# cafferychen777/flashdeconv

Measured on AMD Instinct MI355X. Metric: spots/sec to convergence (1M x 2000 x 30), higher is better.
Workload: dtype f64

## Files before the change

### flashdeconv_amd/csrc/bcd_sweep_inst.cpp

```cpp
#include <algorithm>
#include <cstdlib>
#include "bcd_device.h"
#include "fdx_graph.h"

#ifndef FDX_PART
#error "compile with -DFDX_PART=<n> -DFDX_K_LO=<lo> -DFDX_K_HI=<hi>"
#endif

namespace fdx {

constexpr int sweep_chunk(int K) {
#ifdef FDX_KC_OVERRIDE
    return K < FDX_KC_OVERRIDE ? K : FDX_KC_OVERRIDE;
#endif
    return K < 8 ? K : K <= 29 ? 8 : K <= 33 ? 7 : K <= 37 ? 6 : K <= 41 ? 5 : K <= 45 ? 4 : K <= 49 ? 3 : K <= 51 ? 2 : K <= 64 ? 8 : K <= 72 ? 6 : K <= 88 ? 4 : K <= 96 ? 2 : 8;
}

template <int K, int KC>
__global__ __launch_bounds__(256) void bcd_sweep_kernel(
    const double* __restrict__ H, const double* __restrict__ XtX, const double* __restrict__ beta_in,
    double* __restrict__ beta_out, const int* __restrict__ ell_base, const int* __restrict__ slice_off,
    const int* __restrict__ deg, unsigned long long* __restrict__ stats, double* __restrict__ rel_change,
    const double lambda, const double rho, const double tol, const int ldh, const int ld_, const int n,
    const int n_slices, const int it) {
    const int lane = threadIdx.x & 63;
    const int wib = __builtin_amdgcn_readfirstlane(threadIdx.x >> 6);

    if (it > 0) {
        const double rc = fold_rel_change(stats + (size_t)(it - 1) * 128, lane);
        if (blockIdx.x == 0 && threadIdx.x == 0) rel_change[it - 1] = rc;
        if (rc < tol) return;
    }

    const int slice = xcd_remap(blockIdx.x, gridDim.x) * 4 + wib;
    if (slice >= n_slices) return;
    const int i = min(slice * 64 + lane, n - 1);
    const size_t ld = (size_t)ld_;

    const int w0 = slice_off[slice];
    const int w = slice_off[slice + 1] - w0;

    double b[K];
#pragma unroll
    for (int k = 0; k < K; ++k) b[k] = beta_in[k * ld + i];
    const int* ell = ell_base + (size_t)w0 * 64 + (i & 63);
    const int dg = deg[i];
    const double lam_deg = lambda * (double)dg;
    const double lam_eff = (dg > 0) ? lambda : 0.0;

    double dmax = 0.0, amax = 0.0;
#pragma unroll
    for (int kc = 0; kc < K; kc += KC) {
        double c[KC];
#pragma unroll
        for (int q = 0; q < KC; ++q) c[q] = 0.0;
#pragma unroll 2
        for (int m = 0; m < w; ++m) {
            const int j = ell[(size_t)m * 64];
#pragma unroll
            for (int q = 0; q < KC; ++q)
                if (kc + q < K) c[q] += beta_in[(kc + q) * ld + j];
        }
#pragma unroll
        for (int q = 0; q < KC; ++q) {
            const int k = kc + q;
            if (k < K) {
                const double h = H[k * (size_t)ldh + i];
                const double* g = XtX + k * K;
                double r0 = 0.0, r1 = 0.0;
#pragma unroll
                for (int j = 0; j + 1 < K; j += 2) {
                    r0 = fma(g[j], b[j], r0);
                    r1 = fma(g[j + 1], b[j + 1], r1);
                }
                if (K & 1) r0 = fma(g[K - 1], b[K - 1], r0);
                const double gkk = g[k];
                const double old = b[k];
                const double res = (h - (r0 + r1) + gkk * old) + lam_eff * c[q];
                const double den = gkk + lam_deg;
                const double st = res > rho ? res - rho : (res < -rho ? res + rho : 0.0);
                const double qv = fmax(0.0, st / den);
                const double nw = (den > 1e-10) ? qv : 0.0;
                dmax = fmax(dmax, fabs(nw - old));
                amax = fmax(amax, fabs(old));
                b[k] = nw;
                beta_out[k * ld + i] = nw;
            }
        }
    }
    dmax = wave_max(dmax);
    amax = wave_max(amax);
    if (lane == 0) {
        unsigned long long* s = stats + (size_t)it * 128;
        const int slot = slice & 63;
        atomicMax(s + slot, (unsigned long long)__double_as_longlong(dmax));
        atomicMax(s + 64 + slot, (unsigned long long)__double_as_longlong(amax));
    }
}

__device__ __forceinline__ const char __attribute__((address_space(1)))* plane_base(const double* p) {
    unsigned long long v = (unsigned long long)p;
    asm("" : "+s"(v));
    return (const char __attribute__((address_space(1)))*)v;
}

__device__ __forceinline__ unsigned lane_off(unsigned off) {
    asm("" : "+v"(off));
    return off;
}

#ifndef FDX_SWEEP_WPE
#define FDX_SWEEP_WPE 1
#endif
template <int K, int KC, bool OBJ, bool QUAD = true, bool INIT = false>
__global__ __launch_bounds__(256, ((OBJ && K > 40 && K <= 64) || (K > 64 && K <= 96)) ? 2 : (OBJ ? 1 : FDX_SWEEP_WPE)) void bcd_sweep_tiled_kernel(
    const double* __restrict__ H, const double* __restrict__ XtX, const double* __restrict__ beta_in,
    double* __restrict__ beta_out, const unsigned short* __restrict__ ell_local, const int* __restrict__ slice_off,
    const int* __restrict__ deg, const int* __restrict__ tile_halo, const int* __restrict__ tile_hcnt,
    unsigned long long* __restrict__ stats, double* __restrict__ rel_change, const double lambda, const double rho,
    const double tol, const int ldh, const int ld_, const int n, const int S, const int it,
    const int* __restrict__ tile_list, const double init_v, const int* __restrict__ send_head, const int4* __restrict__ send_ent,
    double* __restrict__ send_buf) {
    extern __shared__ __attribute__((aligned(16))) double lds[];
    const int tid = threadIdx.x;
    const int lane = tid & 63;
    const int tile = tile_list ? tile_list[xcd_remap(blockIdx.x, gridDim.x)] : xcd_remap(blockIdx.x, gridDim.x);
    const bool real = (tile * 256 + tid) < n;
    const int i = min(tile * 256 + tid, n - 1);
    const size_t ld = (size_t)ld_;
    const int slice = __builtin_amdgcn_readfirstlane(i >> 6);
    const int w0 = slice_off[slice];
    const int w = slice_off[slice + 1] - w0;
    const int Ht = tile_hcnt[tile];
    const int* halo = tile_halo + (size_t)tile * FDX_TILE_HALO_CAP;
    const int dg = deg[i];
    int hidx0 = halo[tid];
    if (!OBJ && it > 0) {
        const double rc = fold_rel_change(stats + (size_t)(it - 1) * 128, lane);
        if (blockIdx.x == 0 && tid == 0) rel_change[it - 1] = rc;
        asm volatile("" :: "v"(dg), "v"(hidx0), "s"(w0), "s"(w), "s"(Ht));
        if (rc < tol) return;
    }
    hidx0 = (tid < Ht) ? hidx0 : 0;

    const unsigned ioff = (unsigned)i * 8u, hoff = (unsigned)hidx0 * 8u;
#define PLANE_AT(base, off) (*(const double __attribute__((address_space(1)))*)(plane_base(base) + lane_off(off)))
    double b[K];
#pragma unroll
    for (int k = 0; k < K; ++k) b[k] = INIT ? init_v : PLANE_AT(beta_in + k * ld, ioff);
    const unsigned short* ell = ell_local + (size_t)w0 * 64 + (i & 63);
    const double lam_deg = lambda * (double)dg;
    const double lam_eff = (dg > 0) ? lambda : 0.0;
    unsigned slots[8];
    const unsigned zslot = (unsigned)(256 + Ht);
#pragma unroll
    for (int m2 = 0; m2 < 8; ++m2) {
        unsigned lo = (unsigned)__builtin_nontemporal_load(&ell[(size_t)(2 * m2) * 64]);
        unsigned hi = (unsigned)__builtin_nontemporal_load(&ell[(size_t)(2 * m2 + 1) * 64]);
        lo = (2 * m2 < w) ? lo : zslot;
        hi = (2 * m2 + 1 < w) ? hi : zslot;
        slots[m2] = lo | (hi << 16);
    }
    double hv[KC], hreg[KC];
#pragma unroll
    for (int q = 0; q < KC; ++q) {
        hv[q] = INIT ? init_v : PLANE_AT(beta_in + q * ld, hoff);
        hreg[q] = __builtin_nontemporal_load(&PLANE_AT(H + q * (size_t)ldh, ioff));
    }

    double dmax = 0.0, amax = 0.0;
    double o_cross = 0.0, o_quad = 0.0, o_spat = 0.0, o_l1 = 0.0;
#pragma unroll
    for (int kc = 0; kc < K; kc += KC) {
#pragma unroll
        for (int q = 0; q < KC; ++q)
            if (kc + q < K) lds[q * S + tid] = b[kc + q];
        if (tid < Ht) {
#pragma unroll
            for (int q = 0; q < KC; ++q)
                if (kc + q < K) lds[q * S + 256 + tid] = hv[q];
        }
        for (int h = tid + 256; h < Ht; h += 256) {
            const int j = halo[h];
#pragma unroll
            for (int q = 0; q < KC; ++q)
                if (kc + q < K) lds[q * S + 256 + h] = INIT ? init_v : beta_in[(kc + q) * ld + j];
        }
        if (tid < KC) lds[tid * S + 256 + Ht] = 0.0;
        __syncthreads();
        double c[KC];
#pragma unroll
        for (int q = 0; q < KC; ++q) c[q] = 0.0;
#pragma unroll
        for (int m4 = 0; m4 < 16; m4 += 4) {
            if (m4 < w) {
#pragma unroll
                for (int m = m4; m < m4 + 4; ++m) {
                    const int slot = (int)((slots[m >> 1] >> (16 * (m & 1))) & 0xffffu);
#pragma unroll
                    for (int q = 0; q < KC; ++q)
                        if (kc + q < K) c[q] += lds[q * S + slot];
                }
            }
        }
        for (int m = 16; m < w; ++m) {
            const int slot = ell[(size_t)m * 64];
#pragma unroll
            for (int q = 0; q < KC; ++q)
                if (kc + q < K) c[q] += lds[q * S + slot];
        }
        __syncthreads();
#pragma unroll
        for (int q = 0; q < KC; ++q) {
            const int k = kc + q;
            if (k < K) {
                const double h = hreg[q];
                const double* g = XtX + k * K;
                double r0 = 0.0, r1 = 0.0;
                if (!OBJ || QUAD) {
#pragma unroll
                    for (int j = 0; j + 1 < K; j += 2) {
                        r0 = fma(g[j], b[j], r0);
                        r1 = fma(g[j + 1], b[j + 1], r1);
                    }
                    if (K & 1) r0 = fma(g[K - 1], b[K - 1], r0);
                }
                const double gkk = (!OBJ || QUAD) ? g[k] : 0.0;
                const double old = b[k];
                if (OBJ) {
                    o_cross = fma(old, h, o_cross);
                    if (QUAD) o_quad = fma(old, r0 + r1, o_quad);
                    o_spat = fma(old, (double)dg * old - c[q], o_spat);
                    o_l1 += fabs(old);
                    asm volatile("" : "+v"(o_quad));
                } else {
                    const double res = (h - (r0 + r1) + gkk * old) + lam_eff * c[q];
                    const double den = gkk + lam_deg;
                    const double st = res > rho ? res - rho : (res < -rho ? res + rho : 0.0);
                    const double qv = fmax(0.0, st / den);
                    const double nw = (den > 1e-10) ? qv : 0.0;
                    dmax = fmax(dmax, fabs(nw - old));
                    amax = fmax(amax, fabs(old));
                    b[k] = nw;
                    __builtin_nontemporal_store(nw, (double __attribute__((address_space(1)))*)(plane_base(beta_out + k * ld) + lane_off(ioff)));
                }
            }
            if (kc + KC < K) {
#pragma unroll
                for (int t = 2 * q; t < 2 * q + 2; ++t) {
                    const int j = t < KC ? t : t - KC;
                    if (kc + KC + j < K) {
                        if (t < KC) { if (!INIT) hv[j] = PLANE_AT(beta_in + (kc + KC + j) * ld, hoff); }
                        else hreg[j] = __builtin_nontemporal_load(&PLANE_AT(H + (kc + KC + j) * (size_t)ldh, ioff));
                    }
                }
                __builtin_amdgcn_sched_barrier(0);
            }
        }
    }
    if (OBJ) {
        if (!real) { o_cross = o_quad = o_spat = o_l1 = 0.0; }
#pragma unroll
        for (int off = 32; off > 0; off >>= 1) {
            o_cross += __shfl_xor(o_cross, off, 64);
            o_quad += __shfl_xor(o_quad, off, 64);
            o_spat += __shfl_xor(o_spat, off, 64);
            o_l1 += __shfl_xor(o_l1, off, 64);
        }
        __syncthreads();
        if (lane == 0) { lds[(tid >> 6) * 4 + 0] = o_cross; lds[(tid >> 6) * 4 + 1] = o_quad; lds[(tid >> 6) * 4 + 2] = o_spat; lds[(tid >> 6) * 4 + 3] = o_l1; }
        __syncthreads();
        if (tid < 4) rel_change[(size_t)tile * 4 + tid] = ((lds[tid] + lds[4 + tid]) + lds[8 + tid]) + lds[12 + tid];
        return;
    }
    if (!OBJ && send_head != nullptr) {
        int hd = real ? send_head[i] : 0;
        while (hd != 0) {
            const int4 e = send_ent[hd - 1];
            double* o = send_buf + (size_t)K * e.x + e.z;
#pragma unroll
            for (int k = 0; k < K; ++k) o[(size_t)k * e.y] = b[k];
            hd = e.w;
        }
    }
    dmax = wave_max(dmax);
    amax = wave_max(amax);
    if (lane == 0) {
        unsigned long long* s = stats + (size_t)it * 128;
        const int slot = slice & 63;
        atomicMax(s + slot, (unsigned long long)__double_as_longlong(dmax));
        atomicMax(s + 64 + slot, (unsigned long long)__double_as_longlong(amax));
    }
}

template <int K>
static void launch_k(const BcdSweepArgs& a, hipStream_t st) {
    if (a.tiled) {
        constexpr int KC = sweep_chunk(K);
        const int S = 256 + a.halo_max + 1;
        const size_t lds = (size_t)KC * S * sizeof(double);
        if (lds <= 64 * 1024 && (long long)a.ld * 8 < (1LL << 32) && (long long)a.ldh * 8 < (1LL << 32)) {
            if (a.objective) {
                if constexpr (K > 64) {
                    hipLaunchKernelGGL((bcd_sweep_tiled_kernel<K, KC, true, false>), dim3(a.n_tiles), dim3(256), lds, st, a.H, a.XtX,
                                       a.beta_in, a.beta_out, a.ell_local, a.slice_off, a.deg, a.tile_halo, a.tile_hcnt,
                                       a.stats, a.rel_change, a.lambda, a.rho, a.tol, a.ldh, a.ld, a.n, S, a.it, nullptr, 0.0, a.send_head, a.send_ent, a.send_buf);
                } else {
                    hipLaunchKernelGGL((bcd_sweep_tiled_kernel<K, KC, true>), dim3(a.n_tiles), dim3(256), lds, st, a.H, a.XtX,
                                       a.beta_in, a.beta_out, a.ell_local, a.slice_off, a.deg, a.tile_halo, a.tile_hcnt,
                                       a.stats, a.rel_change, a.lambda, a.rho, a.tol, a.ldh, a.ld, a.n, S, a.it, nullptr, 0.0, a.send_head, a.send_ent, a.send_buf);
                }
            }
            else if (a.tile_list) {
                if (a.n_list > 0)
                    hipLaunchKernelGGL((bcd_sweep_tiled_kernel<K, KC, false>), dim3(a.n_list), dim3(256), lds, st, a.H, a.XtX,
                                       a.beta_in, a.beta_out, a.ell_local, a.slice_off, a.deg, a.tile_halo, a.tile_hcnt,
                                       a.stats, a.rel_change, a.lambda, a.rho, a.tol, a.ldh, a.ld, a.n, S, a.it, a.tile_list, 0.0, a.send_head, a.send_ent, a.send_buf);
            } else if (a.init_uniform != 0.0) {
                if constexpr (K <= 64) {
                    hipLaunchKernelGGL((bcd_sweep_tiled_kernel<K, KC, false, true, true>), dim3(a.n_tiles), dim3(256), lds, st, a.H, a.XtX,
                                       a.beta_in, a.beta_out, a.ell_local, a.slice_off, a.deg, a.tile_halo, a.tile_hcnt,
                                       a.stats, a.rel_change, a.lambda, a.rho, a.tol, a.ldh, a.ld, a.n, S, a.it, nullptr, a.init_uniform, a.send_head, a.send_ent, a.send_buf);
                }
            } else {
                hipLaunchKernelGGL((bcd_sweep_tiled_kernel<K, KC, false>), dim3(a.n_tiles), dim3(256), lds, st, a.H, a.XtX,
                                   a.beta_in, a.beta_out, a.ell_local, a.slice_off, a.deg, a.tile_halo, a.tile_hcnt,
                                   a.stats, a.rel_change, a.lambda, a.rho, a.tol, a.ldh, a.ld, a.n, S, a.it, nullptr, 0.0, a.send_head, a.send_ent, a.send_buf);
            }
            return;
        }
    }
    const int nblk = ceil_div(a.n_slices, 4);
    hipLaunchKernelGGL((bcd_sweep_kernel<K, sweep_chunk(K)>), dim3(nblk), dim3(256), 0, st, a.H, a.XtX, a.beta_in,
                       a.beta_out, a.ell, a.slice_off, a.deg, a.stats, a.rel_change, a.lambda, a.rho, a.tol, a.ldh,
                       a.ld, a.n, a.n_slices, a.it);
}

#ifndef FDX_K_STEP
#define FDX_K_STEP 1
#endif
template <int... Is>
static bool dispatch_range(const BcdSweepArgs& a, hipStream_t st, std::integer_sequence<int, Is...>) {
    bool hit = false;
    (void)std::initializer_list<int>{((a.K == FDX_K_LO + Is * FDX_K_STEP) ? (launch_k<FDX_K_LO + Is * FDX_K_STEP>(a, st), hit = true, 0) : 0)...};
    return hit;
}

#define FDX_CAT2(a, b) a##b
#define FDX_CAT(a, b) FDX_CAT2(a, b)
bool FDX_CAT(bcd_sweep_dispatch_part, FDX_PART)(const BcdSweepArgs& a, hipStream_t st) {
    if (a.K < FDX_K_LO || a.K > FDX_K_HI) return false;
    return dispatch_range(a, st, std::make_integer_sequence<int, (FDX_K_HI - FDX_K_LO) / FDX_K_STEP + 1>{});
}

}
```

### flashdeconv_amd/csrc/finish_kernels.cpp

```cpp
#include "fdx_internal.h"
#include "fdx_kernels.h"

namespace fdx {

__global__ __launch_bounds__(256) void objective_partials_kernel(
    const double* __restrict__ beta, long long ld, const double* __restrict__ H, long long ldh,
    const double* __restrict__ XtX, const int* __restrict__ ell_base, const int* __restrict__ slice_off,
    const int* __restrict__ deg, int n, int n_slices, int K, int use_lds, int skip_quad, double* __restrict__ partials) {
    extern __shared__ __attribute__((aligned(16))) double smem[];
    __shared__ double red[4][4];
    const int lane = threadIdx.x & 63;
    const int wib = __builtin_amdgcn_readfirstlane(threadIdx.x >> 6);
    const int slice = blockIdx.x * 4 + wib;
    double cross = 0.0, quad = 0.0, spat = 0.0, l1 = 0.0;
    if (slice < n_slices) {
        const int i = slice * 64 + lane;
        const bool active = i < n;
        const int ii = active ? i : n - 1;
        double* tile = smem + (size_t)wib * K * 64;
        if (use_lds)
            for (int k = 0; k < K; ++k) tile[k * 64 + lane] = beta[(size_t)k * ld + ii];
        const int w0 = slice_off[slice];
        const int w = slice_off[slice + 1] - w0;
        const int* ell = ell_base + (size_t)w0 * 64 + lane;
        const double dg = (double)deg[ii];
        for (int k = 0; k < K; ++k) {
            const double bk = use_lds ? tile[k * 64 + lane] : beta[(size_t)k * ld + ii];
            double nb = 0.0;
            for (int m = 0; m < w; ++m) nb += beta[(size_t)k * ld + ell[(size_t)m * 64]];
            double gb = 0.0;
            const double* g = XtX + (size_t)k * K;
            if (!skip_quad)
                for (int l = 0; l < K; ++l) gb = fma(g[l], use_lds ? tile[l * 64 + lane] : beta[(size_t)l * ld + ii], gb);
            cross = fma(bk, H[(size_t)k * ldh + ii], cross);
            quad = fma(bk, gb, quad);
            spat = fma(bk, dg * bk - nb, spat);
            l1 += fabs(bk);
        }
        if (!active) { cross = quad = spat = l1 = 0.0; }
    }
#pragma unroll
    for (int off = 32; off > 0; off >>= 1) {
        cross += __shfl_xor(cross, off, 64);
        quad += __shfl_xor(quad, off, 64);
        spat += __shfl_xor(spat, off, 64);
        l1 += __shfl_xor(l1, off, 64);
    }
    if (lane == 0) { red[wib][0] = cross; red[wib][1] = quad; red[wib][2] = spat; red[wib][3] = l1; }
    __syncthreads();
    if (threadIdx.x < 4) {
        const int o = threadIdx.x;
        partials[(size_t)blockIdx.x * 4 + o] = ((red[0][o] + red[1][o]) + red[2][o]) + red[3][o];
    }
}

__global__ __launch_bounds__(256) void normalize_export_kernel(const double* __restrict__ beta, long long ld,
                                                               const int* __restrict__ perm, int n, int n_slices, int K,
                                                               int use_lds, double* __restrict__ beta_out,
                                                               double* __restrict__ prop_out) {
    extern __shared__ __attribute__((aligned(16))) double smem[];
    __shared__ double inv_s[4][64];
    __shared__ int row_s[4][64];
    const int lane = threadIdx.x & 63;
    const int wib = __builtin_amdgcn_readfirstlane(threadIdx.x >> 6);
    const int slice = blockIdx.x * 4 + wib;
    if (slice >= n_slices) return;
    const int i = slice * 64 + lane;
    const bool active = i < n;
    const int ii = active ? i : n - 1;
    const int Ks = K | 1;
    double* tile = smem + (size_t)wib * Ks * 64;
    double s = 0.0;
    for (int k = 0; k < K; ++k) {
        const double v = beta[(size_t)k * ld + ii];
        s += v;
        if (use_lds) tile[lane * Ks + k] = v;
    }
    const double den = (s < 1e-10) ? 1e-10 : s;
    const int orow = perm ? perm[ii] : ii;
    if (!use_lds) {
        if (active)
            for (int k = 0; k < K; ++k) {
                const double v = beta[(size_t)k * ld + ii];
                if (beta_out) beta_out[(size_t)orow * K + k] = v;
                if (prop_out) prop_out[(size_t)orow * K + k] = (s == 0.0) ? 1.0 / (double)K : v / den;
            }
        return;
    }
    inv_s[wib][lane] = (s == 0.0) ? -1.0 : den;
    row_s[wib][lane] = active ? orow : -1;
    __builtin_amdgcn_s_waitcnt(0xc07f);
    const int total = 64 * K;
    const int ds = 64 / K, dk = 64 - ds * K;
    int sp = lane / K, k = lane - sp * K;
    const double inv_K = 1.0 / (double)K;
    for (int f = lane; f < total; f += 64) {
        const int row = row_s[wib][sp];
        if (row >= 0) {
            const double v = tile[sp * Ks + k];
            const double dd = inv_s[wib][sp];
            if (beta_out) __builtin_nontemporal_store(v, beta_out + (size_t)row * K + k);
            if (prop_out) __builtin_nontemporal_store((dd < 0.0) ? inv_K : v / dd, prop_out + (size_t)row * K + k);
        }
        sp += ds;
        k += dk;
        if (k >= K) { k -= K; ++sp; }
    }
}

template <bool LDS_TILE>
__global__ __launch_bounds__(256) void spot_diagnostics_kernel(
    const double* __restrict__ beta, long long ld, const double* __restrict__ H, long long ldh,
    const double* __restrict__ XtX, int ldg, const double* __restrict__ row_sq, const int* __restrict__ ell_base,
    const int* __restrict__ slice_off, const int* __restrict__ deg, const int* __restrict__ perm, int n, int n_slices, int K,
    double* __restrict__ out) {
    extern __shared__ __attribute__((aligned(16))) double smem[];
    const int lane = threadIdx.x & 63;
    const int wib = __builtin_amdgcn_readfirstlane(threadIdx.x >> 6);
    const int slice = blockIdx.x * 4 + wib;
    if (slice >= n_slices) return;
    const int i = slice * 64 + lane;
    const bool active = i < n;
    const int ii = active ? i : n - 1;
    double* tile = smem + (size_t)wib * K * 64;
    if (LDS_TILE)
        for (int k = 0; k < K; ++k) tile[k * 64 + lane] = beta[(size_t)k * ld + ii];
    const int w0 = slice_off[slice];
    const int w = slice_off[slice + 1] - w0;
    const int* ell = ell_base + (size_t)w0 * 64 + lane;
    const int dg = deg[ii];
    auto own = [&](int k) { return LDS_TILE ? tile[k * 64 + lane] : beta[(size_t)k * ld + ii]; };
    double nbr = 0.0;
    int j_next = w > 0 ? ell[0] : 0;
    for (int m = 0; m < w; ++m) {
        const int j = j_next;
        if (m + 1 < w) j_next = ell[(size_t)(m + 1) * 64];
        double a0 = 0.0, a1 = 0.0;
        int k = 0;
#pragma unroll 4
        for (; k + 1 < K; k += 2) {
            const double d0 = own(k) - beta[(size_t)k * ld + j];
            const double d1 = own(k + 1) - beta[(size_t)(k + 1) * ld + j];
            a0 = fma(d0, d0, a0);
            a1 = fma(d1, d1, a1);
        }
        if (k < K) {
            const double d0 = own(k) - beta[(size_t)k * ld + j];
            a0 = fma(d0, d0, a0);
        }
        if (m < dg) nbr += a0 + a1;
    }
    double cross = 0.0, quad = 0.0;
    for (int k = 0; k < K; ++k) {
        const double bk = own(k);
        double gb = 0.0;
        const double* g = XtX + (size_t)k * ldg;
        for (int l = 0; l < K; ++l) gb = fma(g[l], own(l), gb);
        cross = fma(bk, H[(size_t)k * ldh + ii], cross);
        quad = fma(bk, gb, quad);
    }
    if (!active) return;
    const double rs = row_sq[i];
    const size_t o = perm ? (size_t)perm[i] : (size_t)i;
    out[o] = fmax(fma(-2.0, cross, rs) + quad, 0.0);
    out[(size_t)n + o] = rs;
    out[2 * (size_t)n + o] = 0.5 * nbr;
}

static inline size_t tile_lds_bytes(int K) { return (size_t)(K | 1) * 256 * sizeof(double); }
static inline bool tile_fits(int K) { return tile_lds_bytes(K) <= 128 * 1024; }

int objective_partials_count(int n_slices) { return ceil_div(n_slices, 4); }

int launch_objective_partials(const double* beta, long long ld, const double* H, long long ldh, const double* XtX,
                              const int* ell, const int* slice_off, const int* deg, int n, int n_slices, int K,
                              double* partials, hipStream_t st, int skip_quad) {
    if (n <= 0) return 0;
    const int use_lds = tile_fits(K) ? 1 : 0;
    const size_t lds = use_lds ? tile_lds_bytes(K) : 0;
    if (lds > 64 * 1024)
        FDX_HIP(hipFuncSetAttribute((const void*)objective_partials_kernel, hipFuncAttributeMaxDynamicSharedMemorySize, (int)lds));
    hipLaunchKernelGGL(objective_partials_kernel, dim3(ceil_div(n_slices, 4)), dim3(256), lds, st, beta, ld, H, ldh, XtX,
                       ell, slice_off, deg, n, n_slices, K, use_lds, skip_quad, partials);
    FDX_CHECK_LAUNCH();
    return 0;
}

int launch_normalize_export(const double* beta, long long ld, const int* perm, int n, int n_slices, int K,
                            double* beta_out, double* prop_out, hipStream_t st) {
    if (n <= 0) return 0;
    const int use_lds = tile_fits(K) ? 1 : 0;
    const size_t lds = use_lds ? tile_lds_bytes(K) : 0;
    if (lds > 64 * 1024)
        FDX_HIP(hipFuncSetAttribute((const void*)normalize_export_kernel, hipFuncAttributeMaxDynamicSharedMemorySize, (int)lds));
    hipLaunchKernelGGL(normalize_export_kernel, dim3(ceil_div(n_slices, 4)), dim3(256), lds, st, beta, ld, perm, n,
                       n_slices, K, use_lds, beta_out, prop_out);
    FDX_CHECK_LAUNCH();
    return 0;
}

int launch_spot_diagnostics(const double* beta, long long ld, const double* H, long long ldh, const double* XtX, int ldg,
                            const double* row_sq, const int* ell, const int* slice_off, const int* deg, const int* perm, int n,
                            int n_slices, int K, double* out, hipStream_t st) {
    if (n <= 0) return 0;
    const dim3 grid(ceil_div(n_slices, 4));
    if (tile_fits(K)) {
        const size_t lds = (size_t)K * 256 * sizeof(double);
        if (lds > 64 * 1024)
            FDX_HIP(hipFuncSetAttribute((const void*)spot_diagnostics_kernel<true>, hipFuncAttributeMaxDynamicSharedMemorySize, (int)lds));
        hipLaunchKernelGGL(spot_diagnostics_kernel<true>, grid, dim3(256), lds, st, beta, ld, H, ldh, XtX, ldg, row_sq, ell,
                           slice_off, deg, perm, n, n_slices, K, out);
    } else {
        hipLaunchKernelGGL(spot_diagnostics_kernel<false>, grid, dim3(256), 0, st, beta, ld, H, ldh, XtX, ldg, row_sq, ell,
                           slice_off, deg, perm, n, n_slices, K, out);
    }
    FDX_CHECK_LAUNCH();
    return 0;
}

}
```

Before: 278.2 million.

## Raise objective sweep occupancy and unroll normalize-export loads in typed blocks

Changes the launch-bounds minimum waves for the objective sweep so that K up to 51 asks for three waves per EU and K up to 64 asks for two. It also adds asm barriers on the objective accumulators to keep the compiler from reordering them. Separately, the normalize/export kernel is split into LDS and non-LDS template variants and loads beta in compile-time blocks of 16 to raise memory-level parallelism. It also replaces the nontemporal stores with plain stores. The higher occupancy target risks register spills, and switching to plain stores changes how the output writes interact with the cache.

New measurement: 271.6 million. -2.4%, worse.

```diff
diff --git a/flashdeconv_amd/csrc/bcd_sweep_inst.cpp b/flashdeconv_amd/csrc/bcd_sweep_inst.cpp
--- a/flashdeconv_amd/csrc/bcd_sweep_inst.cpp
+++ b/flashdeconv_amd/csrc/bcd_sweep_inst.cpp
@@ -112,8 +112,11 @@
 #ifndef FDX_SWEEP_WPE
 #define FDX_SWEEP_WPE 1
 #endif
+constexpr int sweep_min_waves(int K, bool OBJ) {
+    return (K > 64 && K <= 96) ? 2 : !OBJ ? FDX_SWEEP_WPE : K <= 51 ? 3 : K <= 64 ? 2 : 1;
+}
 template <int K, int KC, bool OBJ, bool QUAD = true, bool INIT = false>
-__global__ __launch_bounds__(256, ((OBJ && K > 40 && K <= 64) || (K > 64 && K <= 96)) ? 2 : (OBJ ? 1 : FDX_SWEEP_WPE)) void bcd_sweep_tiled_kernel(
+__global__ __launch_bounds__(256, sweep_min_waves(K, OBJ)) void bcd_sweep_tiled_kernel(
     const double* __restrict__ H, const double* __restrict__ XtX, const double* __restrict__ beta_in,
     double* __restrict__ beta_out, const unsigned short* __restrict__ ell_local, const int* __restrict__ slice_off,
     const int* __restrict__ deg, const int* __restrict__ tile_halo, const int* __restrict__ tile_hcnt,
@@ -232,6 +235,7 @@
                     if (QUAD) o_quad = fma(old, r0 + r1, o_quad);
                     o_spat = fma(old, (double)dg * old - c[q], o_spat);
                     o_l1 += fabs(old);
+                    asm volatile("" : "+v"(o_cross), "+v"(o_spat), "+v"(o_l1));
                     asm volatile("" : "+v"(o_quad));
                 } else {
                     const double res = (h - (r0 + r1) + gkk * old) + lam_eff * c[q];
diff --git a/flashdeconv_amd/csrc/finish_kernels.cpp b/flashdeconv_amd/csrc/finish_kernels.cpp
--- a/flashdeconv_amd/csrc/finish_kernels.cpp
+++ b/flashdeconv_amd/csrc/finish_kernels.cpp
@@ -1,3 +1,4 @@
+#include <type_traits>
 #include "fdx_internal.h"
 #include "fdx_kernels.h"
 
@@ -54,10 +55,23 @@
     }
 }
 
+template <int N, class F>
+__device__ __forceinline__ void tail_type_block(int rest, int k0, F& f) {
+    if (rest == N) f(k0, std::integral_constant<int, N>{});
+    else if constexpr (N > 1) tail_type_block<N - 1>(rest, k0, f);
+}
+template <int KB, class F>
+__device__ __forceinline__ void for_type_blocks(int K, F f) {
+    int k0 = 0;
+    for (; k0 + KB <= K; k0 += KB) f(k0, std::integral_constant<int, KB>{});
+    if (k0 < K) tail_type_block<KB - 1>(K - k0, k0, f);
+}
+
+constexpr int EXPORT_KB = 16;
+template <bool LDS_TILE>
 __global__ __launch_bounds__(256) void normalize_export_kernel(const double* __restrict__ beta, long long ld,
                                                                const int* __restrict__ perm, int n, int n_slices, int K,
-                                                               int use_lds, double* __restrict__ beta_out,
-                                                               double* __restrict__ prop_out) {
+                                                               double* __restrict__ beta_out, double* __restrict__ prop_out) {
     extern __shared__ __attribute__((aligned(16))) double smem[];
     __shared__ double inv_s[4][64];
     __shared__ int row_s[4][64];
@@ -68,43 +82,66 @@
     const int i = slice * 64 + lane;
     const bool active = i < n;
     const int ii = active ? i : n - 1;
-    const int Ks = K | 1;
-    double* tile = smem + (size_t)wib * Ks * 64;
-    double s = 0.0;
-    for (int k = 0; k < K; ++k) {
-        const double v = beta[(size_t)k * ld + ii];
-        s += v;
-        if (use_lds) tile[lane * Ks + k] = v;
-    }
-    const double den = (s < 1e-10) ? 1e-10 : s;
+    const double* __restrict__ col = beta + ii;
     const int orow = perm ? perm[ii] : ii;
-    if (!use_lds) {
-        if (active)
-            for (int k = 0; k < K; ++k) {
-                const double v = beta[(size_t)k * ld + ii];
-                if (beta_out) beta_out[(size_t)orow * K + k] = v;
-                if (prop_out) prop_out[(size_t)orow * K + k] = (s == 0.0) ? 1.0 / (double)K : v / den;
+    if constexpr (!LDS_TILE) {
+        double s = 0.0;
+        for_type_blocks<EXPORT_KB>(K, [&](int k0, auto nb) {
+            constexpr int N = decltype(nb)::value;
+            double v[N];
+#pragma unroll
+            for (int q = 0; q < N; ++q) v[q] = col[(size_t)(k0 + q) * ld];
+#pragma unroll
+            for (int q = 0; q < N; ++q) s += v[q];
+        });
+        if (!active) return;
+        const double den = (s < 1e-10) ? 1e-10 : s;
+        for_type_blocks<EXPORT_KB>(K, [&](int k0, auto nb) {
+            constexpr int N = decltype(nb)::value;
+            double v[N];
+#pragma unroll
+            for (int q = 0; q < N; ++q) v[q] = col[(size_t)(k0 + q) * ld];
+#pragma unroll
+            for (int q = 0; q < N; ++q) {
+                if (beta_out) beta_out[(size_t)orow * K + k0 + q] = v[q];
+                if (prop_out) prop_out[(size_t)orow * K + k0 + q] = (s == 0.0) ? 1.0 / (double)K : v[q] / den;
             }
+        });
         return;
-    }
-    inv_s[wib][lane] = (s == 0.0) ? -1.0 : den;
-    row_s[wib][lane] = active ? orow : -1;
-    __builtin_amdgcn_s_waitcnt(0xc07f);
-    const int total = 64 * K;
-    const int ds = 64 / K, dk = 64 - ds * K;
-    int sp = lane / K, k = lane - sp * K;
-    const double inv_K = 1.0 / (double)K;
-    for (int f = lane; f < total; f += 64) {
-        const int row = row_s[wib][sp];
-        if (row >= 0) {
-            const double v = tile[sp * Ks + k];
-            const double dd = inv_s[wib][sp];
-            if (beta_out) __builtin_nontemporal_store(v, beta_out + (size_t)row * K + k);
-            if (prop_out) __builtin_nontemporal_store((dd < 0.0) ? inv_K : v / dd, prop_out + (size_t)row * K + k);
-        }
-        sp += ds;
-        k += dk;
-        if (k >= K) { k -= K; ++sp; }
+    } else {
+        const int Ks = K | 1;
+        double* tile = smem + (size_t)wib * Ks * 64;
+        double s = 0.0;
+        for_type_blocks<EXPORT_KB>(K, [&](int k0, auto nb) {
+            constexpr int N = decltype(nb)::value;
+            double v[N];
+#pragma unroll
+            for (int q = 0; q < N; ++q) v[q] = col[(size_t)(k0 + q) * ld];
+#pragma unroll
+            for (int q = 0; q < N; ++q) s += v[q];
+#pragma unroll
+            for (int q = 0; q < N; ++q) tile[lane * Ks + k0 + q] = v[q];
+        });
+        const double den = (s < 1e-10) ? 1e-10 : s;
+        inv_s[wib][lane] = (s == 0.0) ? -1.0 : den;
+        row_s[wib][lane] = active ? orow : -1;
+        __builtin_amdgcn_s_waitcnt(0xc07f);
+        const int total = 64 * K;
+        const int ds = 64 / K, dk = 64 - ds * K;
+        int sp = lane / K, k = lane - sp * K;
+        const double inv_K = 1.0 / (double)K;
+        for (int f = lane; f < total; f += 64) {
+            const int row = row_s[wib][sp];
+            if (row >= 0) {
+                const double v = tile[sp * Ks + k];
+                const double dd = inv_s[wib][sp];
+                if (beta_out) beta_out[(size_t)row * K + k] = v;
+                if (prop_out) prop_out[(size_t)row * K + k] = (dd < 0.0) ? inv_K : v / dd;
+            }
+            sp += ds;
+            k += dk;
+            if (k >= K) { k -= K; ++sp; }
+        }
     }
 }
 
@@ -189,12 +226,16 @@
 int launch_normalize_export(const double* beta, long long ld, const int* perm, int n, int n_slices, int K,
                             double* beta_out, double* prop_out, hipStream_t st) {
     if (n <= 0) return 0;
-    const int use_lds = tile_fits(K) ? 1 : 0;
-    const size_t lds = use_lds ? tile_lds_bytes(K) : 0;
-    if (lds > 64 * 1024)
-        FDX_HIP(hipFuncSetAttribute((const void*)normalize_export_kernel, hipFuncAttributeMaxDynamicSharedMemorySize, (int)lds));
-    hipLaunchKernelGGL(normalize_export_kernel, dim3(ceil_div(n_slices, 4)), dim3(256), lds, st, beta, ld, perm, n,
-                       n_slices, K, use_lds, beta_out, prop_out);
+    const dim3 grid(ceil_div(n_slices, 4));
+    if (tile_fits(K)) {
+        auto kernel = normalize_export_kernel<true>;
+        const size_t lds = tile_lds_bytes(K);
+        if (lds > 64 * 1024)
+            FDX_HIP(hipFuncSetAttribute((const void*)kernel, hipFuncAttributeMaxDynamicSharedMemorySize, (int)lds));
+        hipLaunchKernelGGL(kernel, grid, dim3(256), lds, st, beta, ld, perm, n, n_slices, K, beta_out, prop_out);
+    } else {
+        hipLaunchKernelGGL(normalize_export_kernel<false>, grid, dim3(256), 0, st, beta, ld, perm, n, n_slices, K, beta_out, prop_out);
+    }
     FDX_CHECK_LAUNCH();
     return 0;
 }
```
